# kangxiongbin/HyLight

Measured on AMD Instinct MI355X. Metric: long-read all-vs-all overlaps/sec, higher is better.
Workload: dtype u8/int32

## Files before the change

### hylight_amd/csrc/ava_align.hip

```cpp
#include <algorithm>
#include <memory>
#include <string>
#include <type_traits>
#include <vector>

#include "align_score_setup.h"
#include "ava_internal.h"
#include "dev_prims.h"
#include "wave_ops.h"

namespace hlmi {

namespace {
constexpr int WG = 256;
constexpr int WAVES = WG / 64;
constexpr int SEQ_T_MAX = EXT_MAX + BAND_W;
constexpr int NR_SHORT = 128;
constexpr int WIDE_SHORT = 128;
inline dim3 grid1(size_t n) { return grid_for(n, WG); }

struct Task {
    uint32_t piece;
    uint16_t kind;
    uint16_t narrow;
    uint64_t qa, ta;
    int16_t m, n;
    int16_t dlo;
    int16_t trim;
};
constexpr uint16_t TASK_REV = 4;
constexpr uint16_t TASK_ONE = 8;
struct TaskOut {
    int32_t score;
    int32_t bi, bj;
    uint32_t runs_off, n_runs;
    uint32_t pad;
};
__device__ __forceinline__ uint32_t end_codes(uint32_t first_run, uint32_t last_run) { return (first_run & 15u) | (last_run & 15u) << 4; }

__global__ void piece_task_count_kernel(const Piece *pieces, size_t n, uint32_t *cnt) {
    size_t i = blockIdx.x * (size_t)blockDim.x + threadIdx.x;
    if (i < n) cnt[i] = pieces[i].n_fp + 1;
}

struct TaskRef { uint32_t pk, fp; };
struct PieceGeom {
    uint64_t qo, to;
    uint32_t ql, tl;
    uint32_t strand;
    uint32_t stub_cand;
};
struct TaskGeom {
    const TaskRef *ref;
    const PieceGeom *pg;
    const FixPt *fps;
};
__device__ __forceinline__ Task build_task(const PieceGeom &p, uint32_t piece, uint32_t kind, FixPt f0, FixPt f1, int ext_max) {
    const int ql = (int)p.ql, tl = (int)p.tl;
    const uint64_t qo = p.qo, to = p.to;
    const uint16_t rev = p.strand ? TASK_REV : 0;
    auto qaddr = [&](int pos) { return p.strand ? qo + (uint64_t)(ql - 1 - pos) : qo + (uint64_t)pos; };
    if (kind == 1) {
        const int qs = (int)f0.q, ts = (int)f0.t;
        const int m = qs < ext_max ? qs : ext_max, n2 = ts < m + BAND_W ? ts : m + BAND_W;
        return Task{piece, (uint16_t)(1u | rev), (uint16_t)(qs <= ext_max ? (qs + 1) << 1 : 0), qaddr(qs - 1),
                    to + (uint64_t)(ts - 1), (int16_t)m, (int16_t)n2, (int16_t)(-(BAND_W / 2 - 1)), 0};
    }
    if (kind == 2) {
        const int qe = (int)f0.q, te = (int)f0.t;
        const int m = ql - qe < ext_max ? ql - qe : ext_max, n2 = tl - te < m + BAND_W ? tl - te : m + BAND_W;
        return Task{piece, (uint16_t)(2u | rev), (uint16_t)(ql - qe <= ext_max ? (ql - qe + 1) << 1 : 0), qaddr(qe),
                    to + (uint64_t)te, (int16_t)m, (int16_t)n2, (int16_t)(-(BAND_W / 2 - 1)), 0};
    }
    const int q0 = (int)f0.q, t0 = (int)f0.t, m = (int)f1.q - q0, n2 = (int)f1.t - t0;
    const int delta = n2 - m, ad = delta < 0 ? -delta : delta;
    const bool lng = m > BLOCK_MAX || n2 > BLOCK_MAX;
    const bool narrow = !lng && ad <= NARROW_DELTA;
    const int lw = ad <= HALF_DELTA ? HALF_W : BAND_W;
    return Task{piece, rev, (uint16_t)(narrow ? 1 : 0), qaddr(q0), to + (uint64_t)t0, (int16_t)m, (int16_t)n2,
                (int16_t)((delta < 0 ? delta : 0) - (narrow ? NARROW_PAD : lng ? (lw - 1 - ad) / 2 : BAND_PAD)), 0};
}
__global__ __launch_bounds__(WG) void task_ref_kernel(const Piece *pieces, const uint32_t *task_off, size_t n, const uint32_t *qlen,
                                                       const uint32_t *tlen, const uint64_t *qoff, const uint64_t *toff,
                                                       const FixPt *fps, int stub_oh, int ext_max, TaskRef *task_ref, PieceGeom *pg) {
    const int lane = threadIdx.x & 63;
    const size_t wave = (blockIdx.x * (size_t)blockDim.x + threadIdx.x) >> 6;
    const size_t n_waves = ((size_t)gridDim.x * blockDim.x) >> 6;
    for (size_t i = wave; i < n; i += n_waves) {
        const Piece p = pieces[i];
        const uint32_t n_tasks = p.n_fp + 1;
        TaskRef *out = task_ref + task_off[i];
        for (uint32_t k = (uint32_t)lane; k < n_tasks; k += 64) {
            const uint32_t kind = k == 0 ? 1u : (k == p.n_fp ? 2u : 0u);
            out[k] = TaskRef{(uint32_t)i | kind << 30, p.fp_off + (k == 0 ? 0u : k - 1)};
        }
        if (lane == 0) {
            const uint32_t ql = qlen[p.q], tl = tlen[p.t];
            uint32_t cand = 0;
            if (stub_oh >= 0) {
                const FixPt a = fps[p.fp_off], b = fps[p.fp_off + p.n_fp - 1];
                const uint32_t dq = (uint32_t)(ext_max + stub_oh), dt = (uint32_t)(ext_max + BAND_W + stub_oh);
                cand = ((a.q > dq && a.t > dt) || (ql - b.q > dq && tl - b.t > dt)) ? 1u : 0u;
            }
            pg[i] = PieceGeom{qoff[p.q], toff[p.t], ql, tl, p.strand, cand};
        }
    }
}

__global__ __launch_bounds__(WG) void task_ref_lane_kernel(const Piece *pieces, const uint32_t *task_off, size_t n, const uint32_t *qlen,
                                                            const uint32_t *tlen, const uint64_t *qoff, const uint64_t *toff,
                                                            const FixPt *fps, int stub_oh, int ext_max, TaskRef *task_ref, PieceGeom *pg) {
    const size_t i = blockIdx.x * (size_t)blockDim.x + threadIdx.x;
    if (i >= n) return;
    const Piece p = pieces[i];
    const uint32_t n_tasks = p.n_fp + 1;
    TaskRef *out = task_ref + task_off[i];
    for (uint32_t k = 0; k < n_tasks; ++k) {
        const uint32_t kind = k == 0 ? 1u : (k == p.n_fp ? 2u : 0u);
        out[k] = TaskRef{(uint32_t)i | kind << 30, p.fp_off + (k == 0 ? 0u : k - 1)};
    }
    const uint32_t ql = qlen[p.q], tl = tlen[p.t];
    uint32_t cand = 0;
    if (stub_oh >= 0) {
        const FixPt a = fps[p.fp_off], b = fps[p.fp_off + p.n_fp - 1];
        const uint32_t dq = (uint32_t)(ext_max + stub_oh), dt = (uint32_t)(ext_max + BAND_W + stub_oh);
        cand = ((a.q > dq && a.t > dt) || (ql - b.q > dq && tl - b.t > dt)) ? 1u : 0u;
    }
    pg[i] = PieceGeom{qoff[p.q], toff[p.t], ql, tl, p.strand, cand};
}

struct AlignArgs {
    Task *tasks;
    TaskGeom geom;
    size_t n_tasks;
    const uint32_t *list;
    size_t n_list;
    const uint8_t *qcodes, *tcodes;
    long long q_total, t_total;
    const uint8_t *qpacked, *tpacked;
    const uint32_t *qnflag, *tnflag;
    int match, mismatch, go, ge, ambi;
    int go2, ge2;
    int end_bonus;
    int ext_max;
    int ext_all_long;
    int ungapped;
    int kmax;
    int kgap1;
    int kgap2;
    int one_ok;
    int kext_plain;
    int kext_bonus;
    int trim_ok;
    int kshift;
    TaskOut *out;
    uint32_t *runs;
    uint32_t cap_runs;
    uint32_t *counters;
    uint32_t run_buf_cap;
    uint8_t *cls_bare;
    uint8_t *defer_flag;
    const uint32_t *defer_list, *defer_count;
};

__device__ __forceinline__ uint32_t wave_excl_sum_u32(uint32_t v, int lane, uint32_t &total) {
    (void)lane;
    const uint32_t x = wave_prefix_sum_incl_dpp(v);
    total = (uint32_t)__builtin_amdgcn_readlane((int)x, 63);
    return x - v;
}

constexpr uint32_t RUN_CHUNK = 4096;
constexpr uint32_t RUN_CHUNK_SMALL = 256;
__device__ __forceinline__ uint32_t pool_take(const AlignArgs &a, uint32_t n, uint32_t &chunk_off, uint32_t &chunk_left,
                                              bool &ok, uint32_t chunk = RUN_CHUNK) {
    if (n > chunk_left) {
        const uint32_t want = n > chunk ? n : chunk;
        chunk_off = atomicAdd(&a.counters[0], want);
        chunk_left = want;
        if ((unsigned long long)chunk_off + want > a.cap_runs) { a.counters[1] = 1; chunk_left = 0; ok = false; return 0; }
    }
// ... 72 lines not shown
        v = (v ^ 0x0303030303030303ull) & ~((n >> 1) | (n >> 2));
    }
    return v;
}

__device__ __forceinline__ uint64_t load_window32p(const uint8_t *packed, long long a0, bool down, bool comp, int x) {
    const long long s = down ? a0 - x - 31 : a0 + x;
    const uint8_t *p = packed + (s >> 2);
    uint64_t lo;
    __builtin_memcpy(&lo, p, 8);
    const int sh = 2 * (int)(s & 3);
    uint64_t v = lo >> sh | (uint64_t)p[8] << 1 << (63 - sh);
    if (down) {
        v = __builtin_bitreverse64(v);
        v = (v >> 1 & 0x5555555555555555ull) | (v & 0x5555555555555555ull) << 1;
    }
    return comp ? ~v : v;
}
__device__ __forceinline__ uint32_t ne_bits32(uint64_t q, uint64_t t) {
    const uint64_t d = q ^ t;
    auto even = [](uint32_t x) {
        x = (x | x >> 1) & 0x55555555u;
        x = (x | x >> 1) & 0x33333333u;
        x = (x | x >> 2) & 0x0f0f0f0fu;
        x = (x | x >> 4) & 0x00ff00ffu;
        return (x | x >> 8) & 0xffffu;
    };
    return even((uint32_t)d) | even((uint32_t)(d >> 32)) << 16;
}
__device__ __forceinline__ uint32_t squeeze8(uint64_t f) {
    return (((uint32_t)f * 0x10204080u) >> 28) | (((uint32_t)(f >> 32) * 0x10204080u) >> 28) << 4;
}
__device__ __forceinline__ uint32_t ne_bits8(uint64_t q, uint64_t t) {
    const uint64_t d = q ^ t;
    return squeeze8((d | d >> 1 | d >> 2) & 0x0101010101010101ull);
}
__device__ __forceinline__ uint32_t amb_bits8(uint64_t q, uint64_t t) { return squeeze8((q | t) >> 2 & 0x0101010101010101ull); }
__device__ __forceinline__ bool range_flagged(const uint32_t *nflag, long long lo, long long hi) {
    const uint32_t g0 = (uint32_t)((lo + (long long)DevReads::PAD) >> 5), g1 = (uint32_t)((hi + (long long)DevReads::PAD) >> 5);
    uint32_t any = 0;
    for (uint32_t w = g0 >> 5; w <= g1 >> 5; ++w) {
        uint32_t keep = ~0u;
        if (w == g0 >> 5) keep &= ~0u << (g0 & 31);
        if (w == g1 >> 5) keep &= ~0u >> (31 - (g1 & 31));
        any |= nflag[w] & keep;
    }
    return any != 0;
}
__device__ __forceinline__ bool window_flagged(const uint32_t *nflag, long long a0, bool down, int len) {
    return down ? range_flagged(nflag, a0 - (len - 1), a0) : range_flagged(nflag, a0, a0 + (len - 1));
}

template <int PASS>
__global__ __launch_bounds__(WG) __attribute__((amdgpu_waves_per_eu(PASS == 1 ? 4 : 5))) void classify_kernel(AlignArgs a, uint8_t *cls, unsigned long long *stats) {
    __shared__ unsigned long long s_stat[WAVES][N_ALIGN_STATS];
    constexpr int CMP_WORDS = PASS == 1 ? 64 * (BLOCK_MAX / 32) : 1;
    __shared__ uint32_t s_mm[WAVES][CMP_WORDS], s_up[WAVES][CMP_WORDS], s_dn[WAVES][CMP_WORDS];
    __shared__ uint64_t s_qa[WAVES][PASS == 1 ? 64 : 1], s_ta[WAVES][PASS == 1 ? 64 : 1];
    __shared__ uint32_t s_geo[WAVES][PASS == 1 ? 64 : 1], s_amb[WAVES][2];
    const int lane = threadIdx.x & 63;
    const size_t tid = blockIdx.x * (size_t)blockDim.x + threadIdx.x;
    const size_t n_thr = (size_t)gridDim.x * blockDim.x;
    uint32_t chunk_off = 0, chunk_left = 0;
    uint32_t st[N_ALIGN_STATS] = {};
    const size_t n_units = PASS == 1 ? a.n_tasks : (size_t)*a.defer_count;
    const size_t rounds = (n_units + n_thr - 1) / n_thr;
    TaskRef ref_n{0, 0};
    uint32_t ti_n = 0;
    if (PASS == 1) { if (tid < n_units) ref_n = a.geom.ref[tid]; }
    else if (tid < n_units) ti_n = a.defer_list[tid];
    for (size_t r = 0; r < rounds; ++r) {
        const size_t u = r * n_thr + tid;
        bool live = u < n_units;
        const size_t ti = PASS == 1 || !live ? u : (size_t)ti_n;
        TaskRef ref = ref_n;
        if (PASS == 2 && live) ref = a.geom.ref[ti];
        {
            const size_t un = u + n_thr;
            if (PASS == 1) { if (un < n_units) ref_n = a.geom.ref[un]; }
            else if (un < n_units) ti_n = a.defer_list[un];
        }
        Task tk{};
        bool held = false;
        bool bare = false;
        if (live) {
            const uint32_t pc = ref.pk & 0x3fffffffu, kind = ref.pk >> 30;
            const PieceGeom pg = a.geom.pg[pc];
            held = PASS == 1 && kind != 0 && pg.stub_cand != 0;
            bare = a.cls_bare != nullptr && pg.stub_cand != 0;
            const FixPt f0 = a.geom.fps[ref.fp];
            FixPt f1{0, 0};
            if (kind == 0) f1 = a.geom.fps[ref.fp + 1];
            tk = build_task(pg, pc, kind, f0, f1, a.ext_max);
        }
        const int m = tk.m, n = tk.n;
        uint8_t c = 2;
        bool try_fast = false;
        if (live) {
            if (m <= 0 || n <= 0 || held) c = 0;
            else if ((tk.kind & 3) == 0) {
                if (m > BLOCK_MAX || n > BLOCK_MAX)
                    c = (n > m ? n - m : m - n) <= HALF_DELTA ? CLS_LONG32 : CLS_LONG;
                else { c = tk.narrow ? (m <= NR_SHORT ? 1 : 3) : 2; try_fast = (m == n); }
            } else if ((m < n - tk.dlo ? m : n - tk.dlo) > EXT_MAX) { c = CLS_LONG32; tk.dlo = (int16_t)(-(HALF_W / 2 - 1)); }
            else if (a.ext_all_long) c = CLS_LONG;
            if (c == 2 && (m < n - tk.dlo ? m : n - tk.dlo) <= WIDE_SHORT) c = 4;
        }
        if (PASS == 1 && live) {
            const bool defer = c != 0 && a.kmax >= 0 && ((tk.kind & 3) != 0 || (m != n && c != CLS_LONG && c != CLS_LONG32));
            a.defer_flag[ti] = defer ? 1 : 0;
            if (defer) { live = false; try_fast = false; }
        }
        int k = 0, mpos[3] = {0, 0, 0}, last_x = -1;
        bool ambig = false, shift_ok = false;
        if constexpr (PASS == 1) {
            const int wv = threadIdx.x >> 6;
            bool flagged = false;
            if (try_fast && a.qpacked)
                flagged = window_flagged(a.qnflag, (long long)tk.qa, (tk.kind & TASK_REV) != 0, m) || window_flagged(a.tnflag, (long long)tk.ta, false, m);
            const bool use_packed = a.qpacked != nullptr && __ballot(flagged) == 0;
            uint32_t *mm = s_mm[wv], *mup = s_up[wv], *mdn = s_dn[wv];
            const uint32_t nch = try_fast ? (uint32_t)(m + 31) >> 5 : 0u;
            const uint32_t incl = wave_prefix_sum_incl_dpp(nch), tot = (uint32_t)__builtin_amdgcn_readlane((int)incl, 63);
            const uint32_t st0 = incl - nch;
            if (lane < 2) s_amb[wv][lane] = 0;
            s_qa[wv][lane] = tk.qa; s_ta[wv][lane] = tk.ta;
            auto compare = [&](auto packed_form) {
                constexpr bool PK = decltype(packed_form)::value;
                constexpr int PB = PK ? 32 : 8, PW = 32 / PB;
                constexpr uint32_t FIRST = PK ? 3u : 0xffu;
                using piece_t = std::conditional_t<PK, uint32_t, uint8_t>;
                piece_t *own = (piece_t *)mm, *pm = (piece_t *)mm, *pup = (piece_t *)mup, *pdn = (piece_t *)mdn;
                const uint32_t ptot = tot * PW, pst0 = st0 * PW;
                auto window = [&](bool query, int o, bool rv, int x) {
                    if constexpr (PK) return query ? load_window32p(a.qpacked, (long long)s_qa[wv][o], rv, rv, x) : load_window32p(a.tpacked, (long long)s_ta[wv][o], false, false, x);
                    else return query ? load_window8p(a.qcodes, (long long)s_qa[wv][o], rv, rv, x) : load_window8p(a.tcodes, (long long)s_ta[wv][o], false, false, x);
                };
                for (uint32_t c = (uint32_t)lane; c < ptot; c += 64) own[c] = 0;
                s_geo[wv][lane] = pst0 | (uint32_t)m << 16 | ((tk.kind & TASK_REV) ? 0x80000000u : 0u);
                __builtin_amdgcn_s_waitcnt(0xc07f);
                __builtin_amdgcn_wave_barrier();
                if (nch) own[pst0] = (piece_t)lane;
                __builtin_amdgcn_s_waitcnt(0xc07f);
                __builtin_amdgcn_wave_barrier();
                int carry = 0;
// ... 306 lines not shown
                xs = x; xe = x + 1;
            }
            if (xs >= 0) { runs[nr++] = (uint32_t)(xe - xs) << 4 | OP_X; prev = xe; }
            if (m > prev) runs[nr++] = (uint32_t)(m - prev) << 4 | OP_EQ;
        }
        if (bare) nr = 0;
        uint32_t wave_total;
        const uint32_t mine = wave_excl_sum_u32(nr, lane, wave_total);
        uint32_t base = 0;
        bool ok = true;
        if (wave_total) {
            if (lane == 0) base = pool_take(a, wave_total, chunk_off, chunk_left, ok);
            base = (uint32_t)__shfl((int)base, 0, 64);
            ok = __shfl((int)ok, 0, 64) != 0;
        }
        if (fast) {
            if (ok) for (uint32_t q = 0; q < nr; ++q) a.runs[base + mine + q] = runs[q];
            const bool ext = (tk.kind & 3) != 0;
            const int L = ext_take >= 0 ? ext_take : (m < n ? m : n);
            a.out[ti] = TaskOut{fast_score, ext ? L : m, ext ? L : n, base + mine, ok ? nr : 0, (nr ? end_codes(runs[0], runs[nr - 1]) : 0u) | ext_flag};
        } else if (live && c == 0) {
            a.out[ti] = TaskOut{0, 0, 0, 0, 0, 0};
        }
        int m_dp = m;
        if (live && !fast && (c == 1 || c == 3) && a.kmax >= 0 && last_x >= 0 && a.trim_ok && !a.ungapped) {
            const int mn = m < n ? m : n;
            int T = mn - 1 - last_x;
            T = T < mn - 1 ? T : mn - 1;
            if (T > 0) {
                tk.m = (int16_t)(m - T); tk.n = (int16_t)(n - T); tk.trim = (int16_t)T;
                m_dp = m - T;
                c = m_dp <= NR_SHORT ? 1 : 3;
            }
        }
        if (live) {
            if (a.ungapped && c != 0) c = CLS_UNGAPPED;
            cls[ti] = bare ? 0 : c;
            if (a.cls_bare) a.cls_bare[ti] = bare ? c : 0;
            if (c != 0) a.tasks[ti] = tk;
            if (held) ++st[ST_STUB_EXT];
            else if (m > 0 && n > 0) {
                const uint32_t bases = (uint32_t)(m + n);
                st[ST_BASES] += bases;
                if ((tk.kind & 3) == 0 && m == n) st[ST_BASES_SQUARE] += bases;
                if (c == 0) ++st[ST_FAST];
                else {
                    ++st[ST_DP];
                    if (c == CLS_LONG || c == CLS_LONG32) { ++st[ST_LONG]; st[ST_BASES_LONG] += bases; st[ST_DP_ROWS] += (uint32_t)(m < n - tk.dlo ? m : n - tk.dlo); }
                    else if (c == 2 || c == 4) { st[ST_BASES_WIDE] += bases; st[ST_DP_ROWS] += (uint32_t)(m < n - tk.dlo ? m : n - tk.dlo); }
                    else { st[ST_BASES_NARROW] += bases; st[ST_DP_ROWS] += (uint32_t)m_dp; if (c == 1 && m_dp < NR_SMALL && !bare) ++st[ST_NARROW_SMALL]; }
                }
            }
        }
    }
#pragma unroll
    for (int k = 0; k < N_ALIGN_STATS; ++k) {
        unsigned long long v = st[k];
#pragma unroll
        for (int o = 32; o > 0; o >>= 1) v += __shfl_xor(v, o, 64);
        if (lane == 0) s_stat[threadIdx.x >> 6][k] = v;
    }
    __syncthreads();
    if (threadIdx.x < N_ALIGN_STATS) {
        unsigned long long v = 0;
        for (int w = 0; w < WAVES; ++w) v += s_stat[w][threadIdx.x];
        if (v) atomicAdd(&stats[threadIdx.x], v);
    }
}

__global__ void task_rows_key_kernel(const Task *tasks, const uint32_t *list, size_t n, uint32_t *key) {
    size_t i = blockIdx.x * (size_t)blockDim.x + threadIdx.x;
    if (i < n) key[i] = (uint32_t)tasks[list[i]].m >> 2;
}


__global__ void task_rows_desc_key_kernel(const Task *tasks, const uint32_t *list, size_t n, uint32_t *key) {
    size_t i = blockIdx.x * (size_t)blockDim.x + threadIdx.x;
    if (i >= n) return;
    const Task &t = tasks[list[i]];
    const int rows = (int)t.m < (int)t.n - (int)t.dlo ? (int)t.m : (int)t.n - (int)t.dlo;
    key[i] = 0xffffu - (uint32_t)(rows < 0 ? 0 : rows);
}

constexpr int DP_BIAS = 1 << 24;
constexpr int NT_PAD = 16;
constexpr int NT_EXTRA = NT_PAD + NARROW_DELTA + NARROW_W + 7;
enum { PL_DIAG = 0, PL_EGEF, PL_EEXT, PL_FEXT, PL_NE, N_PLANES };

__device__ __forceinline__ uint32_t shift_in(uint32_t acc, bool bit) {
#if defined(__HIP_DEVICE_COMPILE__)
    const unsigned long long m = __ballot(bit);
    unsigned long long co;
    asm("v_addc_co_u32 %0, %1, %2, %2, %3" : "=v"(acc), "=s"(co) : "v"(acc), "s"(m));
#endif
    return acc;
}

struct NarrowWalk {
    const uint32_t *pl;
    int chunks;
    int lb;
    int m, n, dlo;
    int wmask;
    bool keep_order;
    int trim;
    __device__ __forceinline__ uint32_t word(int plane, int c, int lane) const { return pl[(plane * chunks + c) * 64 + lane]; }
};
struct WalkScore {
    int match, mismatch, go, ge;
    int total;
};
__device__ uint32_t narrow_walk(const NarrowWalk &w, uint32_t *out, uint32_t total, uint32_t *buf = nullptr, uint32_t cap = 0,
                                WalkScore *ws = nullptr, uint32_t *ends = nullptr) {
    int i = w.m, j = w.n, state = 0;
    uint32_t cur_op = OP_EQ, cur_len = (uint32_t)w.trim, n_runs = 0, e_first = 0, e_last = 0;
    auto put = [&]() {
        if (!n_runs) e_first = cur_op;
        e_last = cur_op;
        if (out) out[w.keep_order ? n_runs : total - 1 - n_runs] = cur_len << 4 | cur_op;
// ... 1413 lines not shown
        const bool mrg = first == carry_code;
        carry_code = last;
        if (!WRITE) {
            slots += nr - (mrg ? 1u : 0u);
            continue;
        }
        for (uint32_t x = 0; x < nr; ++x) {
            const uint32_t run = a.runs[r.runs_off + x];
            blen += run >> 4;
            if ((run & 15u) == OP_EQ) nmatch += run >> 4;
            if (x == 0 && mrg) pend += (run >> 4) << 4;
            else {
                if (pend) w[slots++] = pend;
                pend = run;
            }
        }
    }
    if (!WRITE) {
        const bool ok = (slots > 0 || bare) && score >= a.min_dp_score;
        valid[i] = ok ? 1 : 0;
        n_ops[i] = ok ? slots : 0;
        if (a.late) a.late[i] = a.pg[i].stub_cand && !((slots > 0 || bare) && score >= a.stub_score) ? 1 : 0;
        return;
    }
    if (pend) w[slots++] = pend;
    const int qs = (int)fp[0].q - li, ts = (int)fp[0].t - lj;
    const int qe = (int)fp[p.n_fp - 1].q + ri, te = (int)fp[p.n_fp - 1].t + rj;
    const uint32_t ql = a.qlen[p.q];
    PafRec r{};
    r.qid = a.rank_q[p.q]; r.tid = a.rank_t[p.t];
    r.qlen = ql; r.tlen = a.tlen[p.t];
    r.qs = p.strand ? ql - (uint32_t)qe : (uint32_t)qs;
    r.qe = p.strand ? ql - (uint32_t)qs : (uint32_t)qe;
    r.ts = (uint32_t)ts; r.te = (uint32_t)te;
    r.nmatch = (uint32_t)nmatch; r.blen = (uint32_t)blen;
    r.flags = p.strand ? PF_REV : 0;
    r.chunk = a.chunk_of_t[p.t];
    r.cig_off = ops_off[i]; r.cig_n = slots; r.tie = 0;
    recs[i] = r;
    ord_hi[i] = (uint64_t)r.chunk << 32 | p.q;
    ord_lo[i] = (uint64_t)p.t << 43 | (uint64_t)p.strand << 42 | (uint64_t)(p.chain & 0x3fffffu) << 20 | (p.piece & 0xfffffu);
}

__global__ void late_tasks_kernel(const uint32_t *plist, size_t n, const Piece *pieces, const uint32_t *task_off, uint32_t *tasks,
                                  uint32_t *count) {
    size_t j = blockIdx.x * (size_t)blockDim.x + threadIdx.x;
    if (j == 0) *count = (uint32_t)(2 * n);
    if (j >= n) return;
    const uint32_t i = plist[j];
    tasks[2 * j] = task_off[i];
    tasks[2 * j + 1] = task_off[i] + pieces[i].n_fp;
}

__global__ __launch_bounds__(WG) void class_bases_kernel(const uint8_t *cls, const uint8_t *cls_bare, const Task *tasks, size_t n,
                                                          unsigned long long *out) {
    __shared__ unsigned long long s_sum[N_DP_KINDS];
    if (threadIdx.x < N_DP_KINDS) s_sum[threadIdx.x] = 0;
    __syncthreads();
    for (size_t i = blockIdx.x * (size_t)blockDim.x + threadIdx.x; i < n; i += (size_t)gridDim.x * blockDim.x) {
        const int c = cls[i], cb = cls_bare ? cls_bare[i] : 0;
        if (!c && !cb) continue;
        const Task &t = tasks[i];
        int slot;
        if (c) slot = c == 1 ? ((int)t.m < NR_SMALL ? DP_NARROW_SMALL : DP_NARROW) : c == 3 ? DP_NARROW_LONG : c == 2 ? DP_WIDE : c == 4 ? DP_WIDE_SHORT
                  : c == CLS_LONG ? DP_LONG : c == CLS_LONG32 ? DP_LONG32 : DP_UNGAPPED;
        else slot = cb == 1 ? DP_SCORE_NARROW : cb == 3 ? DP_SCORE_NARROW_LONG : cb == 2 ? DP_SCORE_WIDE : cb == 4 ? DP_SCORE_WIDE_SHORT
                  : cb == CLS_LONG ? DP_SCORE_LONG : cb == CLS_LONG32 ? DP_SCORE_LONG32 : DP_UNGAPPED;
        atomicAdd(&s_sum[slot], (unsigned long long)((int)t.m + (int)t.n));
    }
    __syncthreads();
    if (threadIdx.x < N_DP_KINDS && s_sum[threadIdx.x]) atomicAdd(&out[threadIdx.x], s_sum[threadIdx.x]);
}

__global__ __launch_bounds__(WG) void list_ext_kernel(const Task *tasks, const uint32_t *list, size_t n, unsigned long long *out) {
    unsigned long long c = 0, r = 0;
    for (size_t i = blockIdx.x * (size_t)blockDim.x + threadIdx.x; i < n; i += (size_t)gridDim.x * blockDim.x) {
        const Task &t = tasks[list[i]];
        if (t.kind & 3) { ++c; r += (unsigned long long)(int)t.m; }
    }
#pragma unroll
    for (int o = 32; o > 0; o >>= 1) { c += __shfl_xor(c, o, 64); r += __shfl_xor(r, o, 64); }
    if ((threadIdx.x & 63) == 0 && c) { atomicAdd(out, c); atomicAdd(out + 1, r); }
}

__global__ void class_flag_kernel(const uint8_t *cls, size_t n, uint8_t v, uint8_t *flag) {
    size_t i = blockIdx.x * (size_t)blockDim.x + threadIdx.x;
    if (i < n) flag[i] = cls[i] == v ? 1 : 0;
}

__global__ void compact_rows_kernel(const uint32_t *idx, size_t n, const PafRec *recs, const uint64_t *hi,
                                    const uint64_t *lo, PafRec *orecs, uint64_t *ohi, uint64_t *olo) {
    size_t i = blockIdx.x * (size_t)blockDim.x + threadIdx.x;
    if (i >= n) return;
    orecs[i] = recs[idx[i]];
    ohi[i] = hi[idx[i]];
    olo[i] = lo[idx[i]];
}

__global__ __launch_bounds__(WG) void piece_long_flag_kernel(const Piece *pieces, size_t n, const FixPt *fps, const uint32_t *qlen,
                                                              const uint32_t *tlen, int ext_max, uint8_t *flag) {
    const int lane = threadIdx.x & 63;
    const size_t wave = (blockIdx.x * (size_t)blockDim.x + threadIdx.x) >> 6;
    const size_t n_waves = ((size_t)gridDim.x * blockDim.x) >> 6;
    for (size_t i = wave; i < n; i += n_waves) {
        const Piece p = pieces[i];
        const FixPt *fp = fps + p.fp_off;
        bool lng = false;
        if (lane == 0) {
            const FixPt a = fp[0], b = fp[p.n_fp - 1];
            const int ql = (int)qlen[p.q], tl = (int)tlen[p.t];
            auto rows = [&](int aq, int at) {
                const int m = aq < ext_max ? aq : ext_max, nn = at < m + BAND_W ? at : m + BAND_W;
                return m < nn + (BAND_W / 2 - 1) ? m : nn + (BAND_W / 2 - 1);
            };
            lng = rows((int)a.q, (int)a.t) > EXT_MAX || rows(ql - (int)b.q, tl - (int)b.t) > EXT_MAX;
        }
        for (uint32_t k = (uint32_t)lane; k + 1 < p.n_fp && !__any(lng); k += 64) {
            const FixPt f0 = fp[k], f1 = fp[k + 1];
            lng = lng || (int)(f1.q - f0.q) > BLOCK_MAX || (int)(f1.t - f0.t) > BLOCK_MAX;
        }
        const bool any = __any(lng);
        if (lane == 0) flag[i] = any ? 1 : 0;
    }
}
__global__ __launch_bounds__(WG) void piece_long_flag_lane_kernel(const Piece *pieces, size_t n, const FixPt *fps, const uint32_t *qlen,
                                                                   const uint32_t *tlen, int ext_max, uint8_t *flag) {
// ... 153 lines not shown
            launch(L.kind, L.list.p, L.n, ls, L.la, L.blocks);
            if (on_side_) side_launches_ += 1;
        }
        HIP_CHECK(hipGetLastError());
        pending_ = true;
    }
    void join() {
        if (pending_ && on_side_) {
            if (!done_) HIP_CHECK(hipEventCreateWithFlags(&done_, hipEventDisableTiming));
            HIP_CHECK(hipEventRecord(done_, side_stream()));
            HIP_CHECK(hipStreamWaitEvent(stream(), done_, 0));
        }
        pending_ = false;
    }
    double check() {
        double rows_run = 0;
        for (auto &L : launches_) {
            const std::vector<uint32_t> c = L->ctl.download(4);
            if (c[1]) fail(HLMI_EINVAL, "an alignment task exceeds the scratch area of align_long_kernel");
            rows_run += (double)((unsigned long long)c[3] << 32 | c[2]);
        }
        launches_.clear();
        n_started_ = 0;
        return rows_run;
    }

private:
    struct Launch { DpKind kind; size_t n; unsigned blocks; LongArgs la{}; DBuf<uint32_t> list, planes, runs, ctl; };
    std::vector<std::unique_ptr<Launch>> launches_;
    size_t n_started_ = 0;
    const uint32_t chunks_cap_, runs_cap_;
    const int zdrop_;
    const bool on_side_;
    bool pending_ = false;
    hipEvent_t done_ = nullptr;
    double side_launches_ = 0;
};

struct DpExtra {
    const LongArgs *la = nullptr;
    unsigned blocks = 0;
    bool traceback = true;
};

struct AlignPass {
    const AvaInput &in;
    const hlmi_ava_opts &o;
    const PieceSpan &ch;
    const AlignScoreSetup &sc;
    const size_t P, NT;
    const bool small_pieces;
    DBuf<uint32_t> toff, counters, runs, nops, late_idx;
    DBuf<Task> tasks;
    DBuf<TaskRef> task_ref;
    DBuf<PieceGeom> pgeom;
    DBuf<TaskOut> tout;
    DBuf<unsigned long long> astats, lb_bases;
    DBuf<uint8_t> valid, late;
    DBuf<uint8_t> cls, f1, cls_bare, sel_flag;
    DBuf<uint32_t> list1, list2, list3, list4, list_n, sel_list, sel_n;
    AlignArgs aa{};
    AsmArgs as{};
    LongLaunches longs;
    double lb_n[N_DP_KINDS] = {};
    size_t n1 = 0, n2 = 0, n3 = 0, n4 = 0, n_late = 0, n_wide_late = 0, n_bare_tasks = 0, n_long_tb = 0, n_long_bare = 0;
    unsigned long long long_seen = 0;
    double long_rows_run = 0;

    AlignPass(const AvaInput &in_, const hlmi_ava_opts &o_, const uint32_t *d_qlen, const uint32_t *d_tlen, const PieceSpan &ch_,
              const AlignScoreSetup &sc_)
        : in(in_), o(o_), ch(ch_), sc(sc_), P(ch_.n_pieces), NT(ch_.n_fp + ch_.n_pieces),
          small_pieces(NT <= 17 * P && !hook("HLMI_ASM_WAVE")), longs(o_) {
        DBuf<uint32_t> tcnt(P);
        toff.alloc(P);
        hipLaunchKernelGGL(piece_task_count_kernel, grid1(P), dim3(WG), 0, stream(), ch.pieces.p, P, tcnt.p);
        exclusive_scan_u32(tcnt.p, toff.p, P);
        tasks.alloc(NT);
        if (P >= (1u << 30)) fail(HLMI_EINVAL, "more than 2^30 alignment pieces in one batch");
        task_ref.alloc(NT);
        pgeom.alloc(P);
        if (NT <= 17 * P)
            hipLaunchKernelGGL(task_ref_lane_kernel, grid1(P), dim3(WG), 0, stream(), ch.pieces.p, toff.p, P, d_qlen, d_tlen, in.Q->off.p, in.T->off.p,
                               ch.fps.p, o.stub_oh, ext_rows(o), task_ref.p, pgeom.p);
        else
            hipLaunchKernelGGL(task_ref_kernel, dim3((unsigned)std::min<size_t>(cdiv(P, (size_t)WAVES), 256 * 32)), dim3(WG), 0, stream(),
                               ch.pieces.p, toff.p, P, d_qlen, d_tlen, in.Q->off.p, in.T->off.p, ch.fps.p, o.stub_oh, ext_rows(o), task_ref.p, pgeom.p);
        HIP_CHECK(hipGetLastError());
        tout.alloc(NT);
        counters.alloc(2);
        astats.alloc(N_ALIGN_STATS);
        as.pieces = ch.pieces.p; as.fps = ch.fps.p; as.task_off = toff.p; as.tout = tout.p; as.n_pieces = P;
        as.min_dp_score = o.min_dp_score; as.end_bonus = o.end_bonus;
        as.qlen = d_qlen; as.tlen = d_tlen; as.rank_q = in.d_rank_q; as.rank_t = in.d_rank_t; as.chunk_of_t = in.d_chunk_of_t;
        as.pg = pgeom.p; as.stub_score = o.min_dp_score + std::max(0, o.end_bonus);
        as.stage_cap = (uint32_t)ASM_STAGE;
        if (const char *e = hook("HLMI_ASM_STAGE_CAP")) as.stage_cap = (uint32_t)std::min(ASM_STAGE, std::max(0, atoi(e)));
        as.bare = sc.bare ? 1 : 0;
        nops.alloc(P);
        valid.alloc(P);
        late.alloc(o.stub_oh >= 0 ? P : 0);
        late_idx.alloc(o.stub_oh >= 0 ? P : 0);
        sel_n.alloc(1);
        lb_bases.alloc(N_DP_KINDS + 2);
    }

    void begin_attempt(size_t run_share) {
        const size_t open_chunks = MAX_BLOCKS * (4 * WAVES * RUN_CHUNK + 2 * 4 * WAVES * RUN_CHUNK_SMALL) +
                                   (size_t)3 * 256 * 32 * 8 * PK_WAVES * RUN_CHUNK_SMALL;
        const size_t cap_runs = run_share + open_chunks;
        if (cap_runs >= (1ull << 32)) fail(HLMI_ENOMEM, "CIGAR run pool exceeds 4G entries");
        runs.alloc(cap_runs);
        counters.zero();
        lb_bases.zero();
        std::fill(lb_n, lb_n + N_DP_KINDS, 0.0);
        n_bare_tasks = 0;
        aa = AlignArgs{};
        aa.tasks = tasks.p; aa.n_tasks = NT;
        aa.geom = TaskGeom{task_ref.p, pgeom.p, ch.fps.p};
        aa.qcodes = in.Q->codes(); aa.tcodes = in.T->codes();
        aa.q_total = (long long)in.Q->total; aa.t_total = (long long)in.T->total;
        if (!hook("HLMI_CLASSIFY_BYTES")) {
            if (!in.Q->packed_store.p || !in.T->packed_store.p) fail(HLMI_ESTATE, "alignment of a read set without its 2-bit copy (DevReads::pack)");
            aa.qpacked = in.Q->packed(); aa.tpacked = in.T->packed();
            aa.qnflag = in.Q->nflag.p; aa.tnflag = in.T->nflag.p;
        }
        aa.end_bonus = o.end_bonus;
        aa.ext_max = ext_rows(o);
        aa.ext_all_long = sc.ext_all_long ? 1 : 0;
        aa.ungapped = o.bandwidth == 0 ? 1 : 0;
        aa.match = o.match; aa.mismatch = o.mismatch; aa.go = o.gap_open; aa.ge = o.gap_ext; aa.ambi = o.ambi;
        aa.go2 = sc.go2; aa.ge2 = sc.ge2;
        aa.kmax = sc.kmax; aa.kgap1 = sc.kgap1; aa.kgap2 = sc.kgap2; aa.kshift = sc.kshift;
        aa.trim_ok = sc.trim_ok; aa.one_ok = sc.one_ok; aa.kext_plain = sc.kext_plain; aa.kext_bonus = sc.kext_bonus;
        aa.out = tout.p; aa.runs = runs.p; aa.cap_runs = (uint32_t)cap_runs; aa.counters = counters.p;
        as.runs = runs.p;
        aa.run_buf_cap = 0xffffffffu;
        if (const char *e = hook("HLMI_RUN_BUF_CAP")) aa.run_buf_cap = (uint32_t)std::max(0, atoi(e));
        cls.alloc(NT); f1.alloc(NT); cls_bare.alloc(sc.bare ? NT : 0);
        list1.alloc(NT); list2.alloc(NT); list3.alloc(NT); list4.alloc(NT);
        list_n.alloc(4);
        aa.cls_bare = sc.bare ? cls_bare.p : nullptr;
    }

    void launch_dp(DpKind k, const uint32_t *list, size_t n, hipStream_t on, const DpExtra &x = {}) {
        if (!n) return;
        aa.list = list; aa.n_list = n;
        lb_n[k] += (double)n;
        KTimer kt(DP_NAMES[k], on);
        switch (k) {
        case DP_NARROW_SMALL: case DP_NARROW: case DP_SCORE_NARROW: case DP_SCORE_NARROW_LONG: launch_narrow(k, aa, sc.packed); break;
        case DP_NARROW_LONG: launch_narrow(k, aa, sc.packed && !hook("HLMI_NARROW_LONG_UNPACKED")); break;
        case DP_WIDE: case DP_WIDE_SHORT: case DP_SCORE_WIDE: case DP_SCORE_WIDE_SHORT: launch_wide(k, aa); break;
        case DP_UNGAPPED: {
            const dim3 grid((unsigned)std::min<size_t>(cdiv(n, (size_t)WG), MAX_BLOCKS));
            if (x.traceback) hipLaunchKernelGGL(align_ungapped_kernel<true>, grid, dim3(WG), 0, stream(), aa, o.zdrop);
            else hipLaunchKernelGGL(align_ungapped_kernel<false>, grid, dim3(WG), 0, stream(), aa, o.zdrop);
            HIP_CHECK(hipGetLastError());
            break;
        }
        case DP_LONG: case DP_LONG32: case DP_SCORE_LONG: case DP_SCORE_LONG32:
            if (!x.la) fail(HLMI_ESTATE, "launch_dp: %s without its scratch areas", DP_NAMES[k]);
            launch_long(k, aa, *x.la, x.blocks, on);
            break;
        default: fail(HLMI_ESTATE, "launch_dp: unknown launch kind %d", (int)k);
        }
    }
    void sum_class_bases() {
        hipLaunchKernelGGL(class_bases_kernel, dim3((unsigned)std::min<size_t>(cdiv(NT, (size_t)WG), 2048)), dim3(WG), 0, stream(), cls.p,
                           sc.bare ? cls_bare.p : nullptr, tasks.p, NT, lb_bases.p);
    }

    void sort_list_by_rows(DBuf<uint32_t> &list, size_t n) {
        if (n < 8) return;
        DBuf<uint32_t> key(n);
        hipLaunchKernelGGL(task_rows_key_kernel, grid1(n), dim3(WG), 0, stream(), tasks.p, list.p, n, key.p);
        sort_pairs_u32_u32(key, list, n, 0, 7);
    }
    std::vector<uint32_t> class_lists(const uint8_t *cls_arr) {
        select_classes4_async(cls_arr, NT, list1.p, list2.p, list3.p, list4.p, list_n.p);
        const std::vector<uint32_t> h = list_n.download(4);
        sort_list_by_rows(list1, h[0]);
        sort_list_by_rows(list3, h[2]);
        return h;
    }
    size_t class_list(const uint8_t *cls_arr, uint8_t v) {
        if (sel_flag.n < NT) { sel_flag.alloc(NT); sel_list.alloc(NT); }
        hipLaunchKernelGGL(class_flag_kernel, grid1(NT), dim3(WG), 0, stream(), cls_arr, NT, v, sel_flag.p);
        select_flagged_indices_async(sel_flag.p, sel_list.p, NT, sel_n.p);
        return (size_t)sel_n.download(1)[0];
    }

    void classify() {
        {
            KTimer kt("align_classify");
            const unsigned nbc = (unsigned)std::min<size_t>(cdiv(NT, (size_t)WG), MAX_BLOCKS);
            astats.zero();
            aa.defer_flag = f1.p;
            aa.defer_list = list1.p; aa.defer_count = list_n.p;
            hipLaunchKernelGGL(classify_kernel<1>, dim3(nbc ? nbc : 1), dim3(WG), 0, stream(), aa, cls.p, astats.p);
            select_flagged_indices_async(f1.p, list1.p, NT, list_n.p);
            hipLaunchKernelGGL(classify_kernel<2>, dim3(std::max(1u, nbc / 4)), dim3(WG), 0, stream(), aa, cls.p, astats.p);
        }
        HIP_CHECK(hipGetLastError());
        sum_class_bases();
        const std::vector<uint32_t> hn = class_lists(cls.p);
        n1 = hn[0]; n2 = hn[1]; n3 = hn[2]; n4 = hn[3];
    }

    size_t prepare_long(const uint8_t *cls_arr, bool tb) {
        if (aa.ungapped) {
            const size_t nl = class_list(cls_arr, CLS_UNGAPPED);
            launch_dp(DP_UNGAPPED, sel_list.p, nl, stream(), {nullptr, 0, tb});
            return nl;
        }
        size_t total = 0;
        for (const bool half : {true, false}) {
            const size_t nl = class_list(cls_arr, half ? CLS_LONG32 : CLS_LONG);
            if (!nl) continue;
            hipLaunchKernelGGL(list_ext_kernel, dim3((unsigned)std::min<size_t>(cdiv(nl, (size_t)WG), 1024)), dim3(WG), 0, stream(), tasks.p,
                               sel_list.p, nl, lb_bases.p + N_DP_KINDS);
            longs.prepare(half ? (tb ? DP_LONG32 : DP_SCORE_LONG32) : (tb ? DP_LONG : DP_SCORE_LONG), tasks.p, sel_list.p, nl);
            total += nl;
        }
        return total;
    }
    void prepare_long_score_only() {
        if (!sc.bare) return;
        const size_t nl = prepare_long(cls_bare.p, false);
        n_bare_tasks += nl; n_long_bare += nl;
    }
    void start_long() {
        longs.start([&](DpKind k, const uint32_t *list, size_t n, hipStream_t on, const LongArgs &la, unsigned blocks) {
            launch_dp(k, list, n, on, {&la, blocks});
        });
    }
    void long_first() {
        long_seen = astats.download(N_ALIGN_STATS)[ST_LONG];
        if (!long_seen && !aa.ungapped) return;
        prepare_long_score_only();
        n_long_tb += prepare_long(cls.p, true);
        start_long();
    }
    bool more_long() { return astats.download(N_ALIGN_STATS)[ST_LONG] > long_seen || aa.ungapped; }

    void run_narrow() {
        size_t n_small = 0;
        if (sc.packed && n1 >= 8) n_small = std::min<size_t>(n1, (size_t)astats.download(N_ALIGN_STATS)[ST_NARROW_SMALL]);
        launch_dp(DP_NARROW_SMALL, list1.p, n_small, stream());
        launch_dp(DP_NARROW, list1.p + n_small, n1 - n_small, stream());
        launch_dp(DP_NARROW_LONG, list3.p, n3, stream());
    }
    void run_wide(size_t n_long, size_t n_short) {
        launch_dp(DP_WIDE, list2.p, n_long, stream());
        launch_dp(DP_WIDE_SHORT, list4.p, n_short, stream());
    }
    void run_score_only(bool with_long) {
        if (!sc.bare) return;
        if (with_long) { prepare_long_score_only(); start_long(); }
        const std::vector<uint32_t> hb = class_lists(cls_bare.p);
        n_bare_tasks += (size_t)hb[0] + hb[1] + hb[2] + hb[3];
        launch_dp(DP_SCORE_NARROW, list1.p, hb[0], stream());
        launch_dp(DP_SCORE_NARROW_LONG, list3.p, hb[2], stream());
        launch_dp(DP_SCORE_WIDE, list2.p, hb[1], stream());
        launch_dp(DP_SCORE_WIDE_SHORT, list4.p, hb[3], stream());
    }

    void late_round() {
        as.plist = nullptr; as.n_pieces = P; as.late = late.p;
        longs.join();
        launch_assemble_count(as, small_pieces, nops.p, valid.p);
        as.late = nullptr;
        n_late = select_flagged_indices(late.p, late_idx.p, P);
        n_wide_late = 0;
        if (!n_late) return;
        hipLaunchKernelGGL(late_tasks_kernel, grid1(n_late), dim3(WG), 0, stream(), late_idx.p, n_late, ch.pieces.p, toff.p, list1.p, list_n.p);
        HIP_CHECK(hipMemsetAsync(cls.p, 0, NT, stream()));
        if (sc.bare) HIP_CHECK(hipMemsetAsync(cls_bare.p, 0, NT, stream()));
        {
            KTimer kt("align_classify");
            aa.defer_list = list1.p; aa.defer_count = list_n.p;
            const unsigned nb2 = (unsigned)std::min<size_t>(cdiv(2 * n_late, (size_t)WG), MAX_BLOCKS);
            hipLaunchKernelGGL(classify_kernel<2>, dim3(nb2 ? nb2 : 1), dim3(WG), 0, stream(), aa, cls.p, astats.p);
        }
        sum_class_bases();
        if (sc.bare) {
            const size_t before = n_bare_tasks;
            run_score_only(more_long());
            n_wide_late = n_bare_tasks - before;
        } else {
            select_classes4_async(cls.p, NT, list1.p, list2.p, list3.p, list4.p, list_n.p);
            const std::vector<uint32_t> hl = list_n.download(4);
            run_wide(hl[1], hl[3]);
            const size_t nl = more_long() ? prepare_long(cls.p, true) : 0;
            start_long();
            n_long_tb += nl;
            n_wide_late = (size_t)hl[1] + hl[3] + nl;
        }
        as.plist = late_idx.p; as.n_pieces = n_late;
        longs.join();
        launch_assemble_count(as, small_pieces, nops.p, valid.p);
        as.plist = nullptr; as.n_pieces = P;
    }

    void report_task_counts() {
        stat_add("align_tasks_narrow", (double)(n1 + n3)); stat_add("align_tasks_wide", (double)(n2 + n4 + (sc.bare ? 0 : n_wide_late)));
        stat_add("align_tasks_score_only", (double)n_bare_tasks);
        stat_add("align_tasks_long", (double)n_long_tb); stat_add("align_tasks_long_score_only", (double)n_long_bare);
    }
    bool end_attempt() {
        HIP_CHECK(hipGetLastError());
        longs.join();
        const std::vector<uint32_t> hc = counters.download(2);
        long_rows_run += longs.check();
        return !hc[1];
    }
    void report_stats() {
        stat_add("align_tasks", (double)NT);
        const std::vector<unsigned long long> h = astats.download(N_ALIGN_STATS);
        stat_add("align_tasks_fast", (double)h[ST_FAST]);
        stat_add("align_tasks_packed", (double)h[ST_PACKED]);
        stat_add("align_tasks_dp", (double)h[ST_DP]);
        stat_add("align_dp_rows", (double)h[ST_DP_ROWS]);
        stat_add("align_dp_bases", (double)h[ST_BASES]);
        stat_add("align_bases_classify", (double)h[ST_BASES_SQUARE]);
        stat_add("align_bases_narrow", (double)h[ST_BASES_NARROW]);
        stat_add("align_bases_wide", (double)h[ST_BASES_WIDE]);
        stat_add("align_bases_long", (double)h[ST_BASES_LONG]);
        const std::vector<unsigned long long> lb = lb_bases.download(N_DP_KINDS + 2);
        stat_add("align_long_rows_run", long_rows_run);
        stat_add("align_long_ext", (double)lb[N_DP_KINDS]);
        stat_add("align_long_ext_rows", (double)lb[N_DP_KINDS + 1]);
        if (longs.on_side()) stat_add("align_long_side_launches", longs.side_launches());
        for (int k = 0; k < N_DP_KINDS; ++k)
            if (lb_n[k] > 0) {
                stat_add(std::string("align_n.") + DP_NAMES[k], lb_n[k]);
                stat_add(std::string("align_bases.") + DP_NAMES[k], (double)lb[k]);
            }
// ... 152 lines not shown
```

Before: 3687.

## Derive task-to-piece mapping from chunk index and fuse class-base sums into classify

Replaces the per-task TaskRef array with a per-64-task chunk_piece index plus task_off lookups. In pass 1 each wave works out which piece every lane belongs to using LDS marks and a prefix max; pass 2 uses a bounded binary search. The separate class_bases_kernel is removed, and per-DP-kind base sums are accumulated inside classify_kernel with wave reductions and atomics. This removes writing and reading a full task-sized array and one full pass over tasks. In exchange, classify does more per-wave work and uses extra LDS.

```diff
diff --git a/hylight_amd/csrc/ava_align.hip b/hylight_amd/csrc/ava_align.hip
--- a/hylight_amd/csrc/ava_align.hip
+++ b/hylight_amd/csrc/ava_align.hip
@@ -43,15 +43,17 @@
     if (i < n) cnt[i] = pieces[i].n_fp + 1;
 }
 
-struct TaskRef { uint32_t pk, fp; };
 struct PieceGeom {
     uint64_t qo, to;
     uint32_t ql, tl;
-    uint32_t strand;
-    uint32_t stub_cand;
+    uint32_t fp_off;
+    uint32_t strand : 1;
+    uint32_t stub_cand : 1;
 };
 struct TaskGeom {
-    const TaskRef *ref;
+    const uint32_t *task_off;
+    const uint32_t *chunk_piece;
+    uint32_t n_pieces;
     const PieceGeom *pg;
     const FixPt *fps;
 };
@@ -80,20 +82,16 @@
     return Task{piece, rev, (uint16_t)(narrow ? 1 : 0), qaddr(q0), to + (uint64_t)t0, (int16_t)m, (int16_t)n2,
                 (int16_t)((delta < 0 ? delta : 0) - (narrow ? NARROW_PAD : lng ? (lw - 1 - ad) / 2 : BAND_PAD)), 0};
 }
-__global__ __launch_bounds__(WG) void task_ref_kernel(const Piece *pieces, const uint32_t *task_off, size_t n, const uint32_t *qlen,
-                                                       const uint32_t *tlen, const uint64_t *qoff, const uint64_t *toff,
-                                                       const FixPt *fps, int stub_oh, int ext_max, TaskRef *task_ref, PieceGeom *pg) {
+__global__ __launch_bounds__(WG) void piece_geom_kernel(const Piece *pieces, const uint32_t *task_off, size_t n, const uint32_t *qlen,
+                                                         const uint32_t *tlen, const uint64_t *qoff, const uint64_t *toff,
+                                                         const FixPt *fps, int stub_oh, int ext_max, uint32_t *chunk_piece, PieceGeom *pg) {
     const int lane = threadIdx.x & 63;
     const size_t wave = (blockIdx.x * (size_t)blockDim.x + threadIdx.x) >> 6;
     const size_t n_waves = ((size_t)gridDim.x * blockDim.x) >> 6;
     for (size_t i = wave; i < n; i += n_waves) {
         const Piece p = pieces[i];
-        const uint32_t n_tasks = p.n_fp + 1;
-        TaskRef *out = task_ref + task_off[i];
-        for (uint32_t k = (uint32_t)lane; k < n_tasks; k += 64) {
-            const uint32_t kind = k == 0 ? 1u : (k == p.n_fp ? 2u : 0u);
-            out[k] = TaskRef{(uint32_t)i | kind << 30, p.fp_off + (k == 0 ? 0u : k - 1)};
-        }
+        const size_t t0 = task_off[i], t1 = t0 + p.n_fp + 1;
+        for (size_t c = (t0 + 63) / 64 + (size_t)lane; c * 64 < t1; c += 64) chunk_piece[c] = (uint32_t)i;
         if (lane == 0) {
             const uint32_t ql = qlen[p.q], tl = tlen[p.t];
             uint32_t cand = 0;
@@ -102,23 +100,19 @@
                 const uint32_t dq = (uint32_t)(ext_max + stub_oh), dt = (uint32_t)(ext_max + BAND_W + stub_oh);
                 cand = ((a.q > dq && a.t > dt) || (ql - b.q > dq && tl - b.t > dt)) ? 1u : 0u;
             }
-            pg[i] = PieceGeom{qoff[p.q], toff[p.t], ql, tl, p.strand, cand};
-        }
-    }
-}
-
-__global__ __launch_bounds__(WG) void task_ref_lane_kernel(const Piece *pieces, const uint32_t *task_off, size_t n, const uint32_t *qlen,
-                                                            const uint32_t *tlen, const uint64_t *qoff, const uint64_t *toff,
-                                                            const FixPt *fps, int stub_oh, int ext_max, TaskRef *task_ref, PieceGeom *pg) {
+            pg[i] = PieceGeom{qoff[p.q], toff[p.t], ql, tl, p.fp_off, p.strand ? 1u : 0u, cand};
+        }
+    }
+}
+
+__global__ __launch_bounds__(WG) void piece_geom_lane_kernel(const Piece *pieces, const uint32_t *task_off, size_t n, const uint32_t *qlen,
+                                                              const uint32_t *tlen, const uint64_t *qoff, const uint64_t *toff,
+                                                              const FixPt *fps, int stub_oh, int ext_max, uint32_t *chunk_piece, PieceGeom *pg) {
     const size_t i = blockIdx.x * (size_t)blockDim.x + threadIdx.x;
     if (i >= n) return;
     const Piece p = pieces[i];
-    const uint32_t n_tasks = p.n_fp + 1;
-    TaskRef *out = task_ref + task_off[i];
-    for (uint32_t k = 0; k < n_tasks; ++k) {
-        const uint32_t kind = k == 0 ? 1u : (k == p.n_fp ? 2u : 0u);
-        out[k] = TaskRef{(uint32_t)i | kind << 30, p.fp_off + (k == 0 ? 0u : k - 1)};
-    }
+    const size_t t0 = task_off[i], t1 = t0 + p.n_fp + 1;
+    for (size_t c = (t0 + 63) / 64; c * 64 < t1; ++c) chunk_piece[c] = (uint32_t)i;
     const uint32_t ql = qlen[p.q], tl = tlen[p.t];
     uint32_t cand = 0;
     if (stub_oh >= 0) {
@@ -126,7 +120,7 @@
         const uint32_t dq = (uint32_t)(ext_max + stub_oh), dt = (uint32_t)(ext_max + BAND_W + stub_oh);
         cand = ((a.q > dq && a.t > dt) || (ql - b.q > dq && tl - b.t > dt)) ? 1u : 0u;
     }
-    pg[i] = PieceGeom{qoff[p.q], toff[p.t], ql, tl, p.strand, cand};
+    pg[i] = PieceGeom{qoff[p.q], toff[p.t], ql, tl, p.fp_off, p.strand ? 1u : 0u, cand};
 }
 
 struct AlignArgs {
@@ -305,8 +299,9 @@
 }
 
 template <int PASS>
-__global__ __launch_bounds__(WG) __attribute__((amdgpu_waves_per_eu(PASS == 1 ? 4 : 5))) void classify_kernel(AlignArgs a, uint8_t *cls, unsigned long long *stats) {
+__global__ __launch_bounds__(WG) __attribute__((amdgpu_waves_per_eu(PASS == 1 ? 4 : 5))) void classify_kernel(AlignArgs a, uint8_t *cls, unsigned long long *stats, unsigned long long *kind_bases) {
     __shared__ unsigned long long s_stat[WAVES][N_ALIGN_STATS];
+    __shared__ unsigned long long s_kind[WAVES][N_DP_KINDS];
     constexpr int CMP_WORDS = PASS == 1 ? 64 * (BLOCK_MAX / 32) : 1;
     __shared__ uint32_t s_mm[WAVES][CMP_WORDS], s_up[WAVES][CMP_WORDS], s_dn[WAVES][CMP_WORDS];
     __shared__ uint64_t s_qa[WAVES][PASS == 1 ? 64 : 1], s_ta[WAVES][PASS == 1 ? 64 : 1];
@@ -318,32 +313,76 @@
     uint32_t st[N_ALIGN_STATS] = {};
     const size_t n_units = PASS == 1 ? a.n_tasks : (size_t)*a.defer_count;
     const size_t rounds = (n_units + n_thr - 1) / n_thr;
-    TaskRef ref_n{0, 0};
+    if (lane < N_DP_KINDS) s_kind[threadIdx.x >> 6][lane] = 0;
+    constexpr uint32_t NO_PIECE = 0xffffffffu;
+    auto wave_pieces = [&](size_t u0, uint32_t &p0, uint32_t &start) {
+        p0 = 0; start = NO_PIECE;
+        if (u0 >= n_units) return;
+        p0 = (uint32_t)__builtin_amdgcn_readfirstlane((int)a.geom.chunk_piece[u0 >> 6]);
+        if (p0 + (uint32_t)lane < a.geom.n_pieces) start = a.geom.task_off[p0 + (uint32_t)lane];
+    };
+    uint32_t p0_n = 0, start_n = NO_PIECE;
     uint32_t ti_n = 0;
-    if (PASS == 1) { if (tid < n_units) ref_n = a.geom.ref[tid]; }
+    if (PASS == 1) wave_pieces(tid - (size_t)lane, p0_n, start_n);
     else if (tid < n_units) ti_n = a.defer_list[tid];
     for (size_t r = 0; r < rounds; ++r) {
         const size_t u = r * n_thr + tid;
         bool live = u < n_units;
         const size_t ti = PASS == 1 || !live ? u : (size_t)ti_n;
-        TaskRef ref = ref_n;
-        if (PASS == 2 && live) ref = a.geom.ref[ti];
+        uint32_t pc = 0, t_first = 0;
+        bool t_last = false;
+        if constexpr (PASS == 1) {
+            const int wv = threadIdx.x >> 6;
+            const uint32_t p0 = p0_n, start = start_n, u0 = (uint32_t)(u - (size_t)lane);
+            wave_pieces(u - (size_t)lane + n_thr, p0_n, start_n);
+            s_geo[wv][lane] = 0;
+            __builtin_amdgcn_s_waitcnt(0xc07f);
+            __builtin_amdgcn_wave_barrier();
+            const uint32_t d = start - u0;
+            if (lane > 0 && start != NO_PIECE && d < 64u) s_geo[wv][d] = (uint32_t)lane;
+            __builtin_amdgcn_s_waitcnt(0xc07f);
+            __builtin_amdgcn_wave_barrier();
+            const int mark = (int)s_geo[wv][lane];
+            __builtin_amdgcn_s_waitcnt(0xc07f);
+            __builtin_amdgcn_wave_barrier();
+            const int rel = wave_prefix_max_incl_dpp(mark);
+            pc = p0 + (uint32_t)rel;
+            t_first = (uint32_t)__shfl((int)start, rel, 64);
+            const bool next_wave_starts = __ballot(lane > 0 && start != NO_PIECE && d == 64u) != 0;
+            t_last = wave_shl1(mark, next_wave_starts ? 1 : 0) != 0 || ti + 1 == a.n_tasks;
+        } else if (live) {
+            const uint32_t P = a.geom.n_pieces, t = (uint32_t)ti;
+            uint32_t lo = a.geom.chunk_piece[ti >> 6];
+            uint32_t next = lo + 1 < P ? a.geom.task_off[lo + 1] : (uint32_t)a.n_tasks;
+            if (next <= t) {
+                uint32_t hi = lo + 65 < P ? lo + 65 : P;
+                ++lo;
+                while (hi - lo > 1) {
+                    const uint32_t mid = lo + (hi - lo) / 2;
+                    if (a.geom.task_off[mid] <= t) lo = mid; else hi = mid;
+                }
+                next = lo + 1 < P ? a.geom.task_off[lo + 1] : (uint32_t)a.n_tasks;
+            }
+            pc = lo;
+            t_first = a.geom.task_off[lo];
+            t_last = next == t + 1;
+        }
         {
             const size_t un = u + n_thr;
-            if (PASS == 1) { if (un < n_units) ref_n = a.geom.ref[un]; }
-            else if (un < n_units) ti_n = a.defer_list[un];
+            if (PASS == 2 && un < n_units) ti_n = a.defer_list[un];
         }
         Task tk{};
         bool held = false;
         bool bare = false;
         if (live) {
-            const uint32_t pc = ref.pk & 0x3fffffffu, kind = ref.pk >> 30;
+            const uint32_t k_in = (uint32_t)ti - t_first, kind = k_in == 0 ? 1u : (t_last ? 2u : 0u);
             const PieceGeom pg = a.geom.pg[pc];
             held = PASS == 1 && kind != 0 && pg.stub_cand != 0;
             bare = a.cls_bare != nullptr && pg.stub_cand != 0;
-            const FixPt f0 = a.geom.fps[ref.fp];
+            const uint32_t fp = pg.fp_off + (k_in == 0 ? 0u : k_in - 1);
+            const FixPt f0 = a.geom.fps[fp];
             FixPt f1{0, 0};
-            if (kind == 0) f1 = a.geom.fps[ref.fp + 1];
+            if (kind == 0) f1 = a.geom.fps[fp + 1];
             tk = build_task(pg, pc, kind, f0, f1, a.ext_max);
         }
         const int m = tk.m, n = tk.n;
@@ -756,6 +795,24 @@
                 }
             }
         }
+        {
+            int kd = -1;
+            if (live && c != 0) {
+                if (bare) kd = c == 1 ? DP_SCORE_NARROW : c == 3 ? DP_SCORE_NARROW_LONG : c == 2 ? DP_SCORE_WIDE : c == 4 ? DP_SCORE_WIDE_SHORT
+                             : c == CLS_LONG ? DP_SCORE_LONG : c == CLS_LONG32 ? DP_SCORE_LONG32 : DP_UNGAPPED;
+                else kd = c == 1 ? ((int)tk.m < NR_SMALL ? DP_NARROW_SMALL : DP_NARROW) : c == 3 ? DP_NARROW_LONG : c == 2 ? DP_WIDE : c == 4 ? DP_WIDE_SHORT
+                        : c == CLS_LONG ? DP_LONG : c == CLS_LONG32 ? DP_LONG32 : DP_UNGAPPED;
+            }
+            const uint32_t kb = kd >= 0 ? (uint32_t)((int)tk.m + (int)tk.n) : 0u;
+            unsigned long long todo = __ballot(kd >= 0);
+            while (todo) {
+                const int kk = __builtin_amdgcn_readlane(kd, __ffsll((long long)todo) - 1);
+                const bool mine = kd == kk;
+                const uint32_t sum = wave_prefix_sum_incl_dpp(mine ? kb : 0u);
+                if (lane == 63) s_kind[threadIdx.x >> 6][kk] += sum;
+                todo &= ~__ballot(mine);
+            }
+        }
     }
 #pragma unroll
     for (int k = 0; k < N_ALIGN_STATS; ++k) {
@@ -769,6 +826,11 @@
         unsigned long long v = 0;
         for (int w = 0; w < WAVES; ++w) v += s_stat[w][threadIdx.x];
         if (v) atomicAdd(&stats[threadIdx.x], v);
+    }
+    if (threadIdx.x < N_DP_KINDS) {
+        unsigned long long v = 0;
+        for (int w = 0; w < WAVES; ++w) v += s_kind[w][threadIdx.x];
+        if (v) atomicAdd(&kind_bases[threadIdx.x], v);
     }
 }
 
@@ -2288,26 +2350,6 @@
     tasks[2 * j + 1] = task_off[i] + pieces[i].n_fp;
 }
 
-__global__ __launch_bounds__(WG) void class_bases_kernel(const uint8_t *cls, const uint8_t *cls_bare, const Task *tasks, size_t n,
-                                                          unsigned long long *out) {
-    __shared__ unsigned long long s_sum[N_DP_KINDS];
-    if (threadIdx.x < N_DP_KINDS) s_sum[threadIdx.x] = 0;
-    __syncthreads();
-    for (size_t i = blockIdx.x * (size_t)blockDim.x + threadIdx.x; i < n; i += (size_t)gridDim.x * blockDim.x) {
-        const int c = cls[i], cb = cls_bare ? cls_bare[i] : 0;
-        if (!c && !cb) continue;
-        const Task &t = tasks[i];
-        int slot;
-        if (c) slot = c == 1 ? ((int)t.m < NR_SMALL ? DP_NARROW_SMALL : DP_NARROW) : c == 3 ? DP_NARROW_LONG : c == 2 ? DP_WIDE : c == 4 ? DP_WIDE_SHORT
-                  : c == CLS_LONG ? DP_LONG : c == CLS_LONG32 ? DP_LONG32 : DP_UNGAPPED;
-        else slot = cb == 1 ? DP_SCORE_NARROW : cb == 3 ? DP_SCORE_NARROW_LONG : cb == 2 ? DP_SCORE_WIDE : cb == 4 ? DP_SCORE_WIDE_SHORT
-                  : cb == CLS_LONG ? DP_SCORE_LONG : cb == CLS_LONG32 ? DP_SCORE_LONG32 : DP_UNGAPPED;
-        atomicAdd(&s_sum[slot], (unsigned long long)((int)t.m + (int)t.n));
-    }
-    __syncthreads();
-    if (threadIdx.x < N_DP_KINDS && s_sum[threadIdx.x]) atomicAdd(&out[threadIdx.x], s_sum[threadIdx.x]);
-}
-
 __global__ __launch_bounds__(WG) void list_ext_kernel(const Task *tasks, const uint32_t *list, size_t n, unsigned long long *out) {
     unsigned long long c = 0, r = 0;
     for (size_t i = blockIdx.x * (size_t)blockDim.x + threadIdx.x; i < n; i += (size_t)gridDim.x * blockDim.x) {
@@ -2567,7 +2609,7 @@
     const bool small_pieces;
     DBuf<uint32_t> toff, counters, runs, nops, late_idx;
     DBuf<Task> tasks;
-    DBuf<TaskRef> task_ref;
+    DBuf<uint32_t> chunk_piece;
     DBuf<PieceGeom> pgeom;
     DBuf<TaskOut> tout;
     DBuf<unsigned long long> astats, lb_bases;
@@ -2592,14 +2634,14 @@
         exclusive_scan_u32(tcnt.p, toff.p, P);
         tasks.alloc(NT);
         if (P >= (1u << 30)) fail(HLMI_EINVAL, "more than 2^30 alignment pieces in one batch");
-        task_ref.alloc(NT);
+        chunk_piece.alloc(cdiv(NT, (size_t)64));
         pgeom.alloc(P);
         if (NT <= 17 * P)
-            hipLaunchKernelGGL(task_ref_lane_kernel, grid1(P), dim3(WG), 0, stream(), ch.pieces.p, toff.p, P, d_qlen, d_tlen, in.Q->off.p, in.T->off.p,
-                               ch.fps.p, o.stub_oh, ext_rows(o), task_ref.p, pgeom.p);
+            hipLaunchKernelGGL(piece_geom_lane_kernel, grid1(P), dim3(WG), 0, stream(), ch.pieces.p, toff.p, P, d_qlen, d_tlen, in.Q->off.p, in.T->off.p,
+                               ch.fps.p, o.stub_oh, ext_rows(o), chunk_piece.p, pgeom.p);
         else
-            hipLaunchKernelGGL(task_ref_kernel, dim3((unsigned)std::min<size_t>(cdiv(P, (size_t)WAVES), 256 * 32)), dim3(WG), 0, stream(),
-                               ch.pieces.p, toff.p, P, d_qlen, d_tlen, in.Q->off.p, in.T->off.p, ch.fps.p, o.stub_oh, ext_rows(o), task_ref.p, pgeom.p);
+            hipLaunchKernelGGL(piece_geom_kernel, dim3((unsigned)std::min<size_t>(cdiv(P, (size_t)WAVES), 256 * 32)), dim3(WG), 0, stream(),
+                               ch.pieces.p, toff.p, P, d_qlen, d_tlen, in.Q->off.p, in.T->off.p, ch.fps.p, o.stub_oh, ext_rows(o), chunk_piece.p, pgeom.p);
         HIP_CHECK(hipGetLastError());
         tout.alloc(NT);
         counters.alloc(2);
@@ -2631,7 +2673,7 @@
         n_bare_tasks = 0;
         aa = AlignArgs{};
         aa.tasks = tasks.p; aa.n_tasks = NT;
-        aa.geom = TaskGeom{task_ref.p, pgeom.p, ch.fps.p};
+        aa.geom = TaskGeom{toff.p, chunk_piece.p, (uint32_t)P, pgeom.p, ch.fps.p};
         aa.qcodes = in.Q->codes(); aa.tcodes = in.T->codes();
         aa.q_total = (long long)in.Q->total; aa.t_total = (long long)in.T->total;
         if (!hook("HLMI_CLASSIFY_BYTES")) {
@@ -2680,11 +2722,6 @@
         default: fail(HLMI_ESTATE, "launch_dp: unknown launch kind %d", (int)k);
         }
     }
-    void sum_class_bases() {
-        hipLaunchKernelGGL(class_bases_kernel, dim3((unsigned)std::min<size_t>(cdiv(NT, (size_t)WG), 2048)), dim3(WG), 0, stream(), cls.p,
-                           sc.bare ? cls_bare.p : nullptr, tasks.p, NT, lb_bases.p);
-    }
-
     void sort_list_by_rows(DBuf<uint32_t> &list, size_t n) {
         if (n < 8) return;
         DBuf<uint32_t> key(n);
@@ -2712,12 +2749,11 @@
             astats.zero();
             aa.defer_flag = f1.p;
             aa.defer_list = list1.p; aa.defer_count = list_n.p;
-            hipLaunchKernelGGL(classify_kernel<1>, dim3(nbc ? nbc : 1), dim3(WG), 0, stream(), aa, cls.p, astats.p);
+            hipLaunchKernelGGL(classify_kernel<1>, dim3(nbc ? nbc : 1), dim3(WG), 0, stream(), aa, cls.p, astats.p, lb_bases.p);
             select_flagged_indices_async(f1.p, list1.p, NT, list_n.p);
-            hipLaunchKernelGGL(classify_kernel<2>, dim3(std::max(1u, nbc / 4)), dim3(WG), 0, stream(), aa, cls.p, astats.p);
+            hipLaunchKernelGGL(classify_kernel<2>, dim3(std::max(1u, nbc / 4)), dim3(WG), 0, stream(), aa, cls.p, astats.p, lb_bases.p);
         }
         HIP_CHECK(hipGetLastError());
-        sum_class_bases();
         const std::vector<uint32_t> hn = class_lists(cls.p);
         n1 = hn[0]; n2 = hn[1]; n3 = hn[2]; n4 = hn[3];
     }
@@ -2795,9 +2831,8 @@
             KTimer kt("align_classify");
             aa.defer_list = list1.p; aa.defer_count = list_n.p;
             const unsigned nb2 = (unsigned)std::min<size_t>(cdiv(2 * n_late, (size_t)WG), MAX_BLOCKS);
-            hipLaunchKernelGGL(classify_kernel<2>, dim3(nb2 ? nb2 : 1), dim3(WG), 0, stream(), aa, cls.p, astats.p);
-        }
-        sum_class_bases();
+            hipLaunchKernelGGL(classify_kernel<2>, dim3(nb2 ? nb2 : 1), dim3(WG), 0, stream(), aa, cls.p, astats.p, lb_bases.p);
+        }
         if (sc.bare) {
             const size_t before = n_bare_tasks;
             run_score_only(more_long());
```

After: 3683. About the same (-0.1%).
